# kakaobrain/rq-vae-transformer

Hardware: AMD Instinct MI355X
Metric: 256x256 images/sec, AR sampling + decode (RQ-Transformer huge, 8x8x4 codes) (higher is better)
Workload: dtype bf16

## Files before the change

### rq-vae-transformer_amd/csrc/conv_halo.hip

```cpp
#include <stdlib.h>
#include <type_traits>
#include "gemm.h"
#include "rq_common.h"
#include "vae_kernels.h"
#ifndef RQ_CONV_NT
#define RQ_CONV_NT 0
#endif
#ifndef RQ_CONVOUT_NT
#define RQ_CONVOUT_NT 0
#endif
static __device__ __forceinline__ rq_u128 ld128_act(const void* p) {
#if RQ_CONV_NT >= 2
    return ld128_nt(p);
#else
    return ld128(p);
#endif
}
static __device__ __forceinline__ void st128_act(void* p, rq_u128 v) {
#if RQ_CONV_NT >= 1
    st128_nt(p, v);
#else
    st128(p, v);
#endif
}

struct ConvHaloArgs {
    const bf16_t* x;
    const bf16_t* w;
    const float* bias;
    const float* gn;
    const bf16_t* resid;
    bf16_t* out;
    float* stats;
    int B, H, W, Cin, Cout;
};

#define RQ_LOG2E 1.4426950408889634f
static __device__ __forceinline__ float rq_silu_l2(float t) { return t * rq_fast_rcp(fmaf(rq_fast_exp2(-t), RQ_LOG2E, RQ_LOG2E)); }

static __device__ __forceinline__ void rq_stats_piece(const rq_u128& u, float (&sum)[4], float (&sq)[4]) {
    const uint32_t w[4] = {u.x, u.y, u.z, u.w};
#pragma unroll
    for (int e = 0; e < 4; ++e) {
        sum[e] = rq_dot2_bf16(w[e], RQ_ONE_X2, sum[e]);
        sq[e] = rq_dot2_bf16(w[e], w[e], sq[e]);
    }
}

constexpr int HT_H = 8, HT_W = 32;
constexpr int HP_W = HT_W + 2;
constexpr int H_BN = 128;
constexpr int HW_BYTES = H_BN * 128;
#ifndef RQ_HALO_WDMA
#define RQ_HALO_WDMA 1
#endif
#ifndef RQ_HALO_PMID
#define RQ_HALO_PMID 0
#endif
#ifndef RQ_HALO_RMID
#define RQ_HALO_RMID 1
#endif
#ifndef RQ_HALO_RES_F32
#define RQ_HALO_RES_F32 1
#endif
constexpr int H_WSLOTS = RQ_HALO_WDMA ? 4 : 3;
constexpr int H_SMEM_BYTES = 2 * (HT_H + 2) * HP_W * 128 + H_WSLOTS * HW_BYTES;
static __device__ __forceinline__ void halo_wait_dma(int nd, int no) {
#define RQ_HC(ND, K) case K: rq_wait_vmcnt_mixed<ND, K>(); break;
#define RQ_HW(ND) switch (no) { RQ_HC(ND, 0) RQ_HC(ND, 1) RQ_HC(ND, 2) RQ_HC(ND, 3) RQ_HC(ND, 4) RQ_HC(ND, 5) RQ_HC(ND, 6) RQ_HC(ND, 7) RQ_HC(ND, 8) \
    RQ_HC(ND, 9) RQ_HC(ND, 10) RQ_HC(ND, 11) RQ_HC(ND, 12) default: rq_wait_vmcnt_mixed<ND, 0>(); break; }
    if (nd >= 2) { RQ_HW(2) } else { RQ_HW(0) }
#undef RQ_HW
#undef RQ_HC
}

template <int PW = HP_W>
static __device__ __forceinline__ unsigned halo_lds_off(int hy, int hx, int c8) {
    return (unsigned)((hy * PW + hx) * 128 + ((c8 ^ ((hx >> 1) & 7)) << 4));
}

#ifdef RQ_CONV_TRACE
__device__ unsigned long long g_conv_trace[8 * 64];
#define RQ_CT(slot) do { if (blockIdx.x == RQ_CONV_TRACE && lane == 0 && (slot) < 64) g_conv_trace[wave * 64 + (slot)] = __builtin_readcyclecounter(); } while (0)
#else
#define RQ_CT(slot) do { } while (0)
#endif
template <int FUSE_GN, int UPS, int RES>
__global__ __launch_bounds__(512, 1) void conv3x3_halo_kernel(ConvHaloArgs p) {
    constexpr bool WDMA = RQ_HALO_WDMA != 0;
    constexpr int TH = HT_H, NTH = 512, RPW = 2, NJ = 2, W_IT = 2, TPX = TH * HT_W, W_SETS = 3, W_SLOTS = H_WSLOTS;
    static_assert(!(FUSE_GN && UPS), "the upsample conv has no Normalize in front of it");
    constexpr int PW = UPS ? HT_W / 2 + 2 : HP_W, PH = UPS ? TH / 2 + 2 : TH + 2;
    constexpr int HP_N = PW * PH;
    constexpr int HALO_BYTES = HP_N * 128;
    constexpr int H_IT = (HP_N * 8 + NTH - 1) / NTH;
    RQ_DYN_SMEM(smem);
    char* sH = (char*)smem;
    char* sW = sH + 2 * HALO_BYTES;
    const int tid = threadIdx.x, lane = tid & 63, wave = tid >> 6;
    const int wm = wave >> 1, wn = wave & 1;
#ifdef RQ_CONV_TRACE
    if (blockIdx.x == RQ_CONV_TRACE && lane == 0) g_conv_trace[wave * 64 + 58] = __builtin_amdgcn_s_memrealtime();
#endif

    const int tiles_x = p.W / HT_W, tiles_y = p.H / TH, NT = p.Cout / H_BN;
    const int n_mt = p.B * tiles_y * tiles_x;
    const int id = blockIdx.x, xcd = id & 7, slot = id >> 3;
    const int per = (n_mt + 7) >> 3;
    const int mtile = xcd * per + slot / NT;
    const int nt = slot - (slot / NT) * NT;
    if (slot >= per * NT || mtile >= n_mt) return;
    const int img = mtile / (tiles_y * tiles_x);
    const int trem = mtile - img * (tiles_y * tiles_x);
    const int ty0 = (trem / tiles_x) * TH, tx0 = (trem - (trem / tiles_x) * tiles_x) * HT_W;
    const int n0 = nt * H_BN;

    const char* gX = (const char*)p.x;
    const char* gWt = (const char*)p.w;
    const int w_row = tid >> 3, w_c8 = tid & 7;
    unsigned w_goff[W_IT];
#pragma unroll
    for (int i = 0; i < W_IT; ++i) w_goff[i] = (unsigned)(((long)(n0 + w_row + (NTH / 8) * i) * 9 * p.Cin + w_c8 * 8) * 2);
    auto load_w = [&](int c, int tap, rq_u128* rw) {
        const unsigned kb = (unsigned)(tap * p.Cin + c * 64) * 2u;
#pragma unroll
        for (int i = 0; i < W_IT; ++i) rw[i] = ld128(gWt + (w_goff[i] + kb));
    };
    rq_u128 rh[H_IT], rw[W_SETS][W_IT], r01[2][W_IT];
    unsigned w_voff[2];
#pragma unroll
    for (int i = 0; i < 2; ++i) {
        const int r = wave * 16 + i * 8 + (lane >> 3);
        w_voff[i] = (unsigned)(((long)(n0 + r) * 9 * p.Cin + ((lane & 7) ^ ((r >> 1) & 7)) * 8) * 2);
    }
    const rq_lds_t sW_dma = rq_lds_addr(sW) + (rq_lds_t)rq_uniform(wave) * 2048u;
    auto dma_w = [&](int c, int tap, unsigned woff) {
        if (tap >= 9) { tap -= 9; ++c; }
        rq_glds16_s2(sW_dma + woff, gWt + (unsigned)rq_uniform((tap * p.Cin + c * 64) * 2), w_voff[0], w_voff[1]);
    };
    if (WDMA) {
        dma_w(0, 0, 0u);
        dma_w(0, 1, (unsigned)HW_BYTES);
        dma_w(0, 2, 2u * HW_BYTES);
    } else {
        load_w(0, 0, r01[0]);
        load_w(0, 1, r01[1]);
        load_w(0, 2, rw[2]);
        load_w(0, 3, rw[0]);
        load_w(0, 4, rw[1]);
    }
    rq_sched_barrier();

    unsigned hd[H_IT];
    const int Hs = UPS ? p.H >> 1 : p.H, Ws = UPS ? p.W >> 1 : p.W;
    const unsigned x_img = (unsigned)((long)img * Hs * Ws * p.Cin * 2) + (unsigned)((tid & 7) * 16);
    const unsigned cin2 = (unsigned)p.Cin * 2u;
    const int hp0 = tid >> 3, hy0 = hp0 / PW, hx0 = hp0 - hy0 * PW;
    {
        int hy = hy0, hx = hx0;
#pragma unroll
        for (int it = 0; it < H_IT; ++it) {
            const int gy = (UPS ? ty0 >> 1 : ty0) + hy - 1, gx = (UPS ? tx0 >> 1 : tx0) + hx - 1;
            const int cy = gy < 0 ? 0 : (gy >= Hs ? Hs - 1 : gy), cx = gx < 0 ? 0 : (gx >= Ws ? Ws - 1 : gx);
            hd[it] = (unsigned)(cy * Ws + cx);
            rh[it] = ld128_act(gX + (x_img + hd[it] * cin2));
            hy += (NTH / 8) / PW; hx += (NTH / 8) % PW;
            if (hx >= PW) { hx -= PW; ++hy; }
        }
    }
    const float* gn = FUSE_GN ? p.gn + (long)img * p.Cin * 2 : nullptr;
    f32x4 gs[4];
    auto load_gs = [&](int c) {
        if (FUSE_GN) {
#pragma unroll
            for (int e = 0; e < 4; ++e) gs[e] = *(const f32x4*)(gn + (c * 64 + (tid & 7) * 8 + e * 2) * 2);
        }
    };
    auto scale_gs = [&]() {
        if (FUSE_GN) {
#pragma unroll
            for (int e = 0; e < 4; ++e) { rq_opaque_f4(gs[e]); gs[e] = gs[e] * RQ_LOG2E; }
        }
    };
    load_gs(0);
    rq_sched_barrier();
    {
        int hp = hp0, hy = hy0, hx = hx0;
        const int c8 = tid & 7;
#pragma unroll
        for (int it = 0; it < H_IT; ++it) {
            const bool in = hp < HP_N;
            const int gy = (UPS ? ty0 >> 1 : ty0) + hy - 1, gx = (UPS ? tx0 >> 1 : tx0) + hx - 1;
            const bool ok = in && gy >= 0 && gy < Hs && gx >= 0 && gx < Ws;
            const unsigned loff16 = in ? halo_lds_off<PW>(hy, hx, c8) >> 4 : 0u;
            hd[it] |= (loff16 << 16) | (ok ? 1u << 29 : 0u) | (in ? 1u << 30 : 0u);
            hp += NTH / 8; hy += (NTH / 8) / PW; hx += (NTH / 8) % PW;
            if (hx >= PW) { hx -= PW; ++hy; }
        }
    }
    auto h_in = [&](int it) { return (hd[it] >> 30) & 1u; };
    auto h_ok = [&](int it) { return (hd[it] >> 29) & 1u; };
    auto h_loff = [&](int it) { return ((hd[it] >> 16) & 0x1fffu) << 4; };
    auto h_goff = [&](int it) { return x_img + (hd[it] & 0xffffu) * cin2; };
    auto load_halo_piece = [&](int c, rq_u128* rh, int it) { rh[it] = ld128_act(gX + (h_goff(it) + (unsigned)c * 128u)); };

    unsigned w_loff[W_IT];
#pragma unroll
    for (int i = 0; i < W_IT; ++i) {
        const int r = w_row + (NTH / 8) * i;
        w_loff[i] = (unsigned)(r * 128 + ((w_c8 ^ ((r >> 1) & 7)) << 4));
    }
    auto halo_piece_value = [&](const rq_u128* rh, int it) -> rq_u128 {
        rq_u128 v = rh[it];
        if (FUSE_GN) {
            float f[8];
            rq_unpack2(v.x, f[0], f[1]);
            rq_unpack2(v.y, f[2], f[3]);
            rq_unpack2(v.z, f[4], f[5]);
            rq_unpack2(v.w, f[6], f[7]);
#pragma unroll
            for (int e = 0; e < 8; e += 2) {
                const f32x4 ss = gs[e >> 1];
                const float a = fmaf(f[e], ss[0], ss[1]), b = fmaf(f[e + 1], ss[2], ss[3]);
                f[e] = rq_silu_l2(a);
                f[e + 1] = rq_silu_l2(b);
            }
            v.x = pack_bf16x2(f[0], f[1]); v.y = pack_bf16x2(f[2], f[3]);
            v.z = pack_bf16x2(f[4], f[5]); v.w = pack_bf16x2(f[6], f[7]);
        }
        if (!h_ok(it)) v = zero128();
        return v;
    };
    auto halo_word = [&](rq_u128* rh, int it, int e) -> uint32_t& { return e == 0 ? rh[it].x : e == 1 ? rh[it].y : e == 2 ? rh[it].z : rh[it].w; };
    auto halo_piece_word = [&](rq_u128* rh, int it, int e) {
        uint32_t& w = halo_word(rh, it, e);
        if (FUSE_GN) {
            const f32x4 ss = gs[e];
            float wlo, whi;
            rq_unpack2(w, wlo, whi);
            const float a = fmaf(wlo, ss[0], ss[1]), b = fmaf(whi, ss[2], ss[3]);
            w = pack_bf16x2(rq_silu_l2(a), rq_silu_l2(b));
        }
        if (!h_ok(it)) w = 0u;
    };
    auto store_w = [&](int wslot, const rq_u128* rw) {
#pragma unroll
        for (int i = 0; i < W_IT; ++i) st128(sW + wslot * HW_BYTES + w_loff[i], rw[i]);
    };

    f32x16 acc[RPW][NJ];
#pragma unroll
    for (int j = 0; j < NJ; ++j)
#pragma unroll
        for (int q = 0; q < 4; ++q) {
            const f32x4 bv = *(const f32x4*)(p.bias + n0 + wn * (NJ * 32) + j * 32 + 8 * q + 4 * (lane >> 5));
#pragma unroll
            for (int i = 0; i < RPW; ++i)
#pragma unroll
                for (int e = 0; e < 4; ++e) acc[i][j][4 * q + e] = bv[e];
        }

    const int ftx = lane & 31, fk = lane >> 5;
    const unsigned rd_w0 = (unsigned)((wn * (NJ * 32) + ftx) * 128 + ((fk ^ ((ftx >> 1) & 7)) << 4));
    unsigned rd_h0[3];
#pragma unroll
    for (int kx = 0; kx < 3; ++kx)
        rd_h0[kx] = UPS ? halo_lds_off<PW>(wm * (RPW / 2), (ftx + kx + 1) >> 1, fk) : halo_lds_off<PW>(wm * RPW, ftx + kx, fk);

    auto load_frags = [&](int hbuf, unsigned woff, int ky, int kx, int ks, bf16x8* af, bf16x8* bfr) {
        const char* hb = sH + ((rd_h0[kx] + (unsigned)(hbuf * HALO_BYTES)) ^ (unsigned)(ks << 5));
        const char* wb = sW + ((rd_w0 ^ (unsigned)(ks << 5)) + woff);
#pragma unroll
        for (int i = 0; i < RPW; ++i) af[i] = as_bf16x8(ld128(hb + (UPS ? (i + ky + 1) >> 1 : i + ky) * (PW * 128)));
#pragma unroll
        for (int j = 0; j < NJ; ++j) bfr[j] = as_bf16x8(ld128(wb + j * (32 * 128)));
    };
#ifndef RQ_HALO_FDEPTH
#define RQ_HALO_FDEPTH 1
#endif
    constexpr int FD = RQ_HALO_FDEPTH, NSET = FD + 1;
    static_assert(FD >= 1 && FD <= 3 && 36 % NSET == 0, "fragment read-ahead of 1..3 k-steps");
    bf16x8 fa[NSET][RPW], fb[NSET][NJ];
    auto mfma_step = [&](int set) {
#pragma unroll
        for (int i = 0; i < RPW; ++i)
#pragma unroll
            for (int j = 0; j < NJ; ++j) acc[i][j] = rq_mfma_32x32x16_bf16(fb[set][j], fa[set][i], acc[i][j]);
    };

    const int NC = p.Cin / 64, last_c = NC - 1;
    auto load_unit = [&](int c, int tap, rq_u128* r) {
        if (tap >= 9) { tap -= 9; ++c; }
        if (c > last_c) return false;
        load_w(c, tap, r);
        return true;
    };
    {
        RQ_CT(0);
        scale_gs();
#pragma unroll
        for (int it = 0; it < H_IT; ++it)
            if (h_in(it)) st128(sH + h_loff(it), halo_piece_value(rh, it));
        if (WDMA) rq_wait_vmcnt_mixed<0, 0>();
        else {
            store_w(0, r01[0]);
            store_w(1, r01[1]);
        }
    }
    rq_syncthreads();
    RQ_CT(1);
#pragma unroll
    for (int g = 0; g < FD; ++g) load_frags(0, 0u, 0, 0, g, fa[g], fb[g]);
    constexpr int CPR = H_BN / 8;
    constexpr int R_IT = TPX * CPR / NTH;
    static_assert(R_IT == 8, "two residual pieces per tap in the first four taps of the last chunk");
    rq_u128 rr[R_IT];
    const bf16_t* rsrc = p.resid;
    static_assert(CPR == 16 && NTH / CPR == HT_W && R_IT == TH, "piece k = tile row k");
    const unsigned io_off0 = (unsigned)((((long)img * p.H + ty0) * p.W + tx0 + (tid >> 4)) * p.Cout + n0 + (tid & 15) * 8) * 2u;
    const unsigned io_step = (unsigned)p.W * (unsigned)p.Cout * 2u;
    auto run_chunk = [&](int c, auto last_tag) {
        constexpr bool LAST = decltype(last_tag)::value;
        const int hbuf = c & 1;
        const unsigned cph = (unsigned)c & 3u;
        auto slot_off = [&](int tap) { return WDMA ? ((cph + (unsigned)tap) & 3u) * (unsigned)HW_BYTES : (unsigned)((tap % 3) * HW_BYTES); };
        constexpr int NPT = H_IT, FIRST = 8 - NPT;
        static_assert(FIRST >= 0, "one patch piece per tap");
#pragma unroll
        for (int tap = 0; tap < 9; ++tap) {
            const int ky = tap / 3, kx = tap - ky * 3;
            const bool have_w2 = !(LAST && tap + 2 >= 9), have_w3 = !(LAST && tap + 3 >= 9);
#ifndef RQ_CONV_ABLATE_STAGE
            if (!WDMA && have_w2) store_w((tap + 2) % 3, rw[(tap + 2) % W_SETS]);
#endif
            if (!WDMA && have_w2) (void)load_unit(c, tap + 5, rw[(tap + 2) % W_SETS]);
            auto n_patch = [&](int t) {
                int n = 0;
                if (!LAST && t >= 0) {
                    if (t == 0 && FUSE_GN) n += 4;
#pragma unroll
                    for (int it = 0; it < H_IT; ++it) n += ((FIRST + it >= 3 ? FIRST + it - 3 : 0) == t) ? 1 : 0;
                }
                return n;
            };
            auto n_resid = [&](int t) { return LAST && RES && t >= 0 && t < R_IT / 2 ? 2 : 0; };
            auto patch_loads = [&]() {
                if (!LAST) {
                    if (tap == 0) load_gs(c + 1);
#pragma unroll
                    for (int it = 0; it < H_IT; ++it) {
                        const int t_use = FIRST + it, t_load = t_use >= 3 ? t_use - 3 : 0;
                        if (t_load == tap) load_halo_piece(c + 1, rh, it);
                    }
                }
            };
            auto resid_loads = [&]() {
                if (LAST && RES && tap < R_IT / 2) {
                    rr[2 * tap] = ld128_act((const char*)rsrc + (io_off0 + (unsigned)(2 * tap) * io_step));
                    rr[2 * tap + 1] = ld128_act((const char*)rsrc + (io_off0 + (unsigned)(2 * tap + 1) * io_step));
                }
            };
            constexpr bool PMID = WDMA && RQ_HALO_PMID, RMID = WDMA && RQ_HALO_RMID;
            if (!PMID) patch_loads();
            if (!RMID) resid_loads();
            const int n_vis = n_patch(tap) + n_resid(tap) + (PMID ? n_patch(tap - 1) : 0) + (RMID ? n_resid(tap - 1) : 0);
            if (!LAST && tap == 1) scale_gs();
            rq_sched_barrier();
            const int pit = tap - FIRST;
            const bool ptap = !LAST && pit >= 0 && pit < H_IT;
            const int pi = ptap ? pit : 0;
#pragma unroll
            for (int ks = 0; ks < 4; ++ks) {
#ifdef RQ_CONV_ABLATE_LDS
                if (false) {}
                else
#endif
#pragma unroll
                for (int i = 0; i < RPW; ++i)
#pragma unroll
                    for (int j = 0; j < NJ; ++j) rq_opaque_acc(acc[i][j]);
                {
                    const int g = tap * 4 + ks + FD, t2 = g >> 2, k2 = g & 3, set2 = g % NSET;
                    if (t2 < 9) load_frags(hbuf, slot_off(t2), t2 / 3, t2 % 3, k2, fa[set2], fb[set2]);
                    else if (!LAST) load_frags(hbuf ^ 1, slot_off(t2), (t2 - 9) / 3, (t2 - 9) % 3, k2, fa[set2], fb[set2]);
                }
                mfma_step((tap * 4 + ks) % NSET);
                if (FUSE_GN && ptap) rq_opaque_u(halo_word(rh, pi, ks));
                if (ptap) halo_piece_word(rh, pi, ks);
                if (FUSE_GN && ptap) rq_opaque_u(halo_word(rh, pi, ks));
                rq_sched_group(0x100, RPW + NJ);
#pragma unroll
                for (int m = 0; m < RPW * NJ; ++m) {
                    rq_sched_group(0x008, 1);
                    if (FUSE_GN && ptap) { rq_sched_group(0x002, 3); rq_sched_group(0x400, 1); }
                }
                rq_sched_barrier();
                if (WDMA && ks == 0) {
                    if (have_w3) dma_w(c, tap + 3, slot_off(tap + 3));
                    if (PMID) patch_loads();
                    if (RMID) resid_loads();
                    rq_sched_barrier();
                }
            }
            if (ptap) { if (h_in(pi)) st128(sH + (hbuf ^ 1) * HALO_BYTES + h_loff(pi), rh[pi]); }
            if (WDMA && have_w2) halo_wait_dma(have_w3 ? 2 : 0, n_vis);
            RQ_CT(2 + (c * 9 + tap) * 2);
            rq_syncthreads();
            RQ_CT(3 + (c * 9 + tap) * 2);
        }
    };
    for (int c = 0; c + 1 < NC; ++c) run_chunk(c, std::false_type{});
    run_chunk(NC - 1, std::true_type{});

    constexpr int LDR = H_BN * 2 + 16;
    static_assert(TPX * LDR + 4096 <= 160 * 1024, "epilogue tile must fit the CU's LDS (the launcher allocates max(staging, epilogue))");
    char* sT = (char*)smem;
    constexpr bool RF32 = RES && RQ_HALO_RES_F32;
    constexpr int LDF = H_BN * 4 + 16;
    static_assert(!RF32 || TPX * LDF <= H_SMEM_BYTES, "the fp32 tile overlays the operand buffers");
    if (RF32) {
#pragma unroll
        for (int i = 0; i < RPW; ++i) {
            const int ml = (wm * RPW + i) * HT_W + (lane & 31);
#pragma unroll
            for (int j = 0; j < NJ; ++j)
#pragma unroll
                for (int q = 0; q < 4; ++q) {
                    const int u = wn * (NJ * 8) + j * 8 + 2 * q + (lane >> 5);
                    f32x4 v;
#pragma unroll
                    for (int e = 0; e < 4; ++e) v[e] = acc[i][j][4 * q + e];
                    *(f32x4*)(sT + ml * LDF + ((u >> 1) + 16 * (u & 1)) * 16) = v;
                }
        }
    }
    if (RES && !RF32) {
#pragma unroll
        for (int k = 0; k < R_IT; ++k) st128(sT + ((tid >> 4) + HT_W * k) * LDR + (tid & 15) * 16, rr[k]);
        rq_syncthreads();
    }
    uint32_t rres[RPW][NJ][4][2];
    if (RES && !RF32) {
#pragma unroll
        for (int i = 0; i < RPW; ++i)
#pragma unroll
            for (int j = 0; j < NJ; ++j)
#pragma unroll
                for (int q = 0; q < 4; ++q) {
                    const int ml = (wm * RPW + i) * HT_W + (lane & 31);
                    const int nl = wn * (NJ * 32) + j * 32 + 8 * q + 4 * (lane >> 5);
                    const uint32_t* rp = (const uint32_t*)(sT + ml * LDR + nl * 2);
                    rres[i][j][q][0] = rp[0];
                    rres[i][j][q][1] = rp[1];
                }
        rq_sched_barrier();
    }
    if (!RF32)
#pragma unroll
    for (int i = 0; i < RPW; ++i) {
        const int ty = wm * RPW + i, tx = lane & 31;
        const int ml = ty * HT_W + tx;
#pragma unroll
        for (int j = 0; j < NJ; ++j) {
#pragma unroll
            for (int q = 0; q < 4; ++q) {
                const int nl = wn * (NJ * 32) + j * 32 + 8 * q + 4 * (lane >> 5);
                float v[4];
#pragma unroll
                for (int e = 0; e < 4; ++e) v[e] = acc[i][j][4 * q + e];
                if (RES && !RF32) {
                    const uint32_t r0 = rres[i][j][q][0], r1 = rres[i][j][q][1];
                    { float lo_, hi_; rq_unpack2(r0, lo_, hi_); v[0] += lo_; v[1] += hi_; }
                    { float lo_, hi_; rq_unpack2(r1, lo_, hi_); v[2] += lo_; v[3] += hi_; }
                }
                struct __attribute__((aligned(8))) u64 { uint32_t a, b; } w2;
                w2.a = pack_bf16x2(v[0], v[1]);
                w2.b = pack_bf16x2(v[2], v[3]);
                *(u64*)(sT + ml * LDR + nl * 2) = w2;
            }
        }
    }
    rq_syncthreads();
    RQ_CT(61);
    float gs_[4], gq_[4];
#pragma unroll
    for (int e = 0; e < 4; ++e) { gs_[e] = 0.f; gq_[e] = 0.f; }
#pragma unroll
    for (int k = 0; k < R_IT; ++k) {
        rq_u128 u;
        if (RF32) {
            const char* src = sT + ((tid >> 4) + HT_W * k) * LDF + (tid & 15) * 16;
            f32x4 a = *(const f32x4*)src, b = *(const f32x4*)(src + 256);
            const rq_u128 r = rr[k];
            { float lo_, hi_; rq_unpack2(r.x, lo_, hi_); a[0] += lo_; a[1] += hi_; }
            { float lo_, hi_; rq_unpack2(r.y, lo_, hi_); a[2] += lo_; a[3] += hi_; }
            { float lo_, hi_; rq_unpack2(r.z, lo_, hi_); b[0] += lo_; b[1] += hi_; }
            { float lo_, hi_; rq_unpack2(r.w, lo_, hi_); b[2] += lo_; b[3] += hi_; }
            u.x = pack_bf16x2(a[0], a[1]); u.y = pack_bf16x2(a[2], a[3]);
            u.z = pack_bf16x2(b[0], b[1]); u.w = pack_bf16x2(b[2], b[3]);
        } else {
            u = ld128(sT + ((tid >> 4) + HT_W * k) * LDR + (tid & 15) * 16);
        }
        st128_act((char*)p.out + (io_off0 + (unsigned)k * io_step), u);
        if (p.stats) rq_stats_piece(u, gs_, gq_);
    }
    if (p.stats) {
        __shared__ float sred[NTH / 64][16][4];
        const int gsz = p.Cout / 32;
        float a0, q0, a1, q1;
        if (gsz == 4) {
            a0 = gs_[0] + gs_[1]; q0 = gq_[0] + gq_[1];
            a1 = gs_[2] + gs_[3]; q1 = gq_[2] + gq_[3];
        } else {
            a0 = (gs_[0] + gs_[1]) + (gs_[2] + gs_[3]);
            q0 = (gq_[0] + gq_[1]) + (gq_[2] + gq_[3]);
            a1 = 0.f; q1 = 0.f;
        }
        a0 += rq_shfl_xor(a0, 16); q0 += rq_shfl_xor(q0, 16); a1 += rq_shfl_xor(a1, 16); q1 += rq_shfl_xor(q1, 16);
        a0 += rq_shfl_xor(a0, 32); q0 += rq_shfl_xor(q0, 32); a1 += rq_shfl_xor(a1, 32); q1 += rq_shfl_xor(q1, 32);
        if (lane < 16) { sred[wave][lane][0] = a0; sred[wave][lane][1] = q0; sred[wave][lane][2] = a1; sred[wave][lane][3] = q1; }
        rq_syncthreads();
        if (wave == 0) {
            const int chunk = (lane >> 1) & 15, pair = lane & 1;
            float a = 0.f, q = 0.f;
#pragma unroll
            for (int w = 0; w < NTH / 64; ++w) { a += sred[w][chunk][pair * 2]; q += sred[w][chunk][pair * 2 + 1]; }
            if (gsz == 16) {
                a += rq_shfl_xor(a, 2);
                q += rq_shfl_xor(q, 2);
            }
            const bool writer = gsz == 4 ? true : (gsz == 8 ? pair == 0 : (pair == 0 && (chunk & 1) == 0));
            if (writer && lane < 32) {
                const int g = (n0 + chunk * 8 + pair * 4) / gsz;
                const int tiles = tiles_x * tiles_y;
                float* o = p.stats + (((long)img * tiles + trem) * 32 + g) * 2;
                o[0] = a;
                o[1] = q;
            }
        }
    }
    RQ_CT(63);
#ifdef RQ_CONV_TRACE
    if (blockIdx.x == RQ_CONV_TRACE && lane == 0) g_conv_trace[wave * 64 + 59] = __builtin_amdgcn_s_memrealtime();
#endif
}

constexpr int PK_SMEM = 160 * 1024;
constexpr int PK_PATCH = (HT_H + 2) * HP_W * 128;
constexpr int PK_P0 = 2 * HW_BYTES;
constexpr int PK_P1 = PK_SMEM - PK_PATCH;
constexpr int PK_PSTRIDE = PK_P1 - PK_P0;
constexpr int PK_LDR = H_BN * 2 + 16;
constexpr int PK_TILE = HT_H * HT_W * PK_LDR;
constexpr int PK_RED = 8 * 16 * 4 * 4;
static_assert(PK_P0 + PK_PATCH + PK_TILE + PK_RED <= PK_SMEM, "epilogue tile over spare + P1");
static_assert(PK_P0 + PK_TILE + PK_RED <= PK_P1, "epilogue tile over P0 + spare");

struct HaloTile { int img, ty0, tx0, n0, trem, cls; };

template <int FUSE_GN, int UPS, int RES>
__global__ __launch_bounds__(512, 1) void conv3x3_halo_pk_kernel(ConvHaloArgs p, int wpx) {
    constexpr int TH = HT_H, NTH = 512, RPW = 2, W_IT = 2, TPX = TH * HT_W;
    constexpr bool SUB = UPS == 2;
    constexpr int TAPS = SUB ? 4 : 9, W_SETS = SUB ? 4 : 3;
    static_assert(!(FUSE_GN && UPS), "the upsample conv has no Normalize in front of it");
    constexpr int PW = UPS == 1 ? HT_W / 2 + 2 : HP_W, PH = UPS == 1 ? TH / 2 + 2 : TH + 2;
    constexpr int HP_N = PW * PH;
    constexpr int H_IT = (HP_N * 8 + NTH - 1) / NTH;
    RQ_DYN_SMEM(smem);
    char* sW = (char*)smem;
    char* sH = (char*)smem + PK_P0;
    const int tid = threadIdx.x, lane = tid & 63, wave = tid >> 6;
    const int wm = wave >> 1, wn = wave & 1;

    const int tiles_x = (SUB ? p.W >> 1 : p.W) / HT_W, tiles_y = (SUB ? p.H >> 1 : p.H) / TH, NT = p.Cout / H_BN;
    constexpr int NCLS = SUB ? 4 : 1;
    const int n_mt = p.B * tiles_y * tiles_x * NCLS;
    const int xcd = blockIdx.x & 7, w0 = blockIdx.x >> 3;
    const int per = (n_mt + 7) >> 3, nslot = per * NT;
    auto slot_ok = [&](int s) { return s < nslot && xcd * per + s / NT < n_mt; };
    auto decode = [&](int s) {
        HaloTile t;
        const int mtile = xcd * per + s / NT;
        t.n0 = (s - (s / NT) * NT) * H_BN;
        const int st = SUB ? mtile >> 2 : mtile;
        t.cls = SUB ? mtile & 3 : 0;
        t.img = st / (tiles_y * tiles_x);
        const int trem = st - t.img * (tiles_y * tiles_x);
        t.trem = trem * NCLS + t.cls;
        t.ty0 = (trem / tiles_x) * TH;
        t.tx0 = (trem - (trem / tiles_x) * tiles_x) * HT_W;
        return t;
    };
    int slot = w0;
    if (!slot_ok(slot)) return;

    unsigned hd[H_IT];
    unsigned x_img = 0;
    const float* gn = nullptr;
    const int Hs = UPS ? p.H >> 1 : p.H, Ws = UPS ? p.W >> 1 : p.W;
    auto set_staging = [&](const HaloTile& t) {
        int tid_s = tid;
        rq_opaque(tid_s);
#pragma unroll
        for (int it = 0; it < H_IT; ++it) {
            const int q = tid_s + NTH * it;
            const int hp = q >> 3, c8 = q & 7;
            const bool in = hp < HP_N;
            const int hy = hp / PW, hx = hp - hy * PW;
            const int gy = (UPS == 1 ? t.ty0 >> 1 : t.ty0) + hy - 1, gx = (UPS == 1 ? t.tx0 >> 1 : t.tx0) + hx - 1;
            const bool ok = in && gy >= 0 && gy < Hs && gx >= 0 && gx < Ws;
            const int cy = gy < 0 ? 0 : (gy >= Hs ? Hs - 1 : gy), cx = gx < 0 ? 0 : (gx >= Ws ? Ws - 1 : gx);
            const unsigned loff16 = in ? halo_lds_off<PW>(hy, hx, c8) >> 4 : 0u;
            hd[it] = (unsigned)(cy * Ws + cx) | (loff16 << 16) | (ok ? 1u << 29 : 0u) | (in ? 1u << 30 : 0u);
        }
        x_img = (unsigned)((long)t.img * Hs * Ws * p.Cin * 2) + (unsigned)((tid & 7) * 16);
        if (FUSE_GN) gn = p.gn + (long)t.img * p.Cin * 2;
    };
    auto restage = [&](const HaloTile& t) {
        int tid_s = tid;
        rq_opaque(tid_s);
        int hp = tid_s >> 3, hy = hp / PW, hx = hp - hy * PW;
#pragma unroll
        for (int it = 0; it < H_IT; ++it) {
            const unsigned in = (hd[it] >> 30) & 1u, lo = hd[it] & 0x1fff0000u;
            const int gy = (UPS == 1 ? t.ty0 >> 1 : t.ty0) + hy - 1, gx = (UPS == 1 ? t.tx0 >> 1 : t.tx0) + hx - 1;
            const bool ok = in && gy >= 0 && gy < Hs && gx >= 0 && gx < Ws;
            const int cy = gy < 0 ? 0 : (gy >= Hs ? Hs - 1 : gy), cx = gx < 0 ? 0 : (gx >= Ws ? Ws - 1 : gx);
// ... 666 lines not shown
bool rq_conv_in_mfma_supported(int H, int W, int Cin, int Cout) {
    return Cin == 3 && Cout == CI_COUT && H % HT_H == 0 && W % HT_W == 0;
}

int rq_launch_conv_in_mfma(const float* x, const float* w, const float* bias, bf16_t* y, float* stats, int B, int H, int W, hipStream_t s) {
    ConvInArgs a{};
    a.x = x; a.w = w; a.bias = bias; a.y = y; a.stats = stats; a.B = B; a.H = H; a.W = W;
    const size_t smem = 4096 + 128 + (size_t)CI_COUT * CI_WROW + 4 * (size_t)CI_STG;
    static RqDeviceOnce attr_once;
    if (attr_once.first()) {
        (void)hipFuncSetAttribute((const void*)conv_in_mfma_kernel, hipFuncAttributeMaxDynamicSharedMemorySize, (int)smem);
    }
    RQ_LAUNCH(conv_in_mfma_kernel, dim3((unsigned)(B * (H / HT_H) * (W / HT_W))), dim3(256), smem, s, a);
    return rq_check_launch("conv_in_mfma_kernel");
}

__global__ __launch_bounds__(256) void gn_params_kernel(const float* part, const float* gamma, const float* beta, float* gn, int B, int HW,
                                                        int C, int nchunk, float eps) {
    __shared__ float sa[8][32], sq[8][32], smean[32], srstd[32];
    const int b = blockIdx.x, tid = threadIdx.x, g = tid & 31, sl = tid >> 5;
    float a = 0.f, q = 0.f;
    for (int c = sl; c < nchunk; c += 8) {
        const float* o = part + (((long)b * nchunk + c) * 32 + g) * 2;
        a += o[0];
        q += o[1];
    }
    sa[sl][g] = a;
    sq[sl][g] = q;
    rq_syncthreads();
    if (tid < 32) {
        float ta = 0.f, tq = 0.f;
#pragma unroll
        for (int k = 0; k < 8; ++k) { ta += sa[k][tid]; tq += sq[k][tid]; }
        const float n = (float)HW * (float)(C / 32);
        const float mean = ta / n;
        float var = tq / n - mean * mean;
        if (var < 0.f) var = 0.f;
        smean[tid] = mean;
        srstd[tid] = 1.0f / sqrtf(var + eps);
    }
    rq_syncthreads();
    const int cpg = C / 32;
    for (int ch = tid; ch < C; ch += 256) {
        const int gg = ch / cpg;
        const float sc = srstd[gg] * gamma[ch];
        gn[((long)b * C + ch) * 2] = sc;
        gn[((long)b * C + ch) * 2 + 1] = beta[ch] - smean[gg] * sc;
    }
}

__global__ void ups_subpixel_weights_kernel(const bf16_t* w, bf16_t* wsub, int Cout, int Cin) {
    const long n = (long)4 * Cout * 4 * Cin;
    const long gid = (long)blockIdx.x * blockDim.x + threadIdx.x;
    if (gid >= n) return;
    const int ci = (int)(gid % Cin);
    long r = gid / Cin;
    const int tap = (int)(r & 3); r >>= 2;
    const int co = (int)(r % Cout);
    const int cls = (int)(r / Cout);
    const int py = cls >> 1, px = cls & 1, a = tap >> 1, b = tap & 1;
    const int ky_lo = py == 0 ? (a == 0 ? 0 : 1) : (a == 0 ? 0 : 2), ky_hi = py == 0 ? (a == 0 ? 0 : 2) : (a == 0 ? 1 : 2);
    const int kx_lo = px == 0 ? (b == 0 ? 0 : 1) : (b == 0 ? 0 : 2), kx_hi = px == 0 ? (b == 0 ? 0 : 2) : (b == 0 ? 1 : 2);
    float acc = 0.f;
    for (int ky = ky_lo; ky <= ky_hi; ++ky)
        for (int kx = kx_lo; kx <= kx_hi; ++kx) acc += bf16_to_f32(w[(((long)co * 3 + ky) * 3 + kx) * Cin + ci]);
    wsub[gid] = f32_to_bf16(acc);
}
int rq_launch_ups_subpixel_weights(const bf16_t* w, bf16_t* wsub, int Cout, int Cin, hipStream_t s) {
    const long n = (long)16 * Cout * Cin;
    RQ_LAUNCH(ups_subpixel_weights_kernel, dim3((unsigned)((n + 255) / 256)), dim3(256), 0, s, w, wsub, Cout, Cin);
    return rq_check_launch("ups_subpixel_weights_kernel");
}
bool rq_conv_halo_subpixel_supported(int H, int W, int Cin, int Cout) {
    return rq_conv_halo_supported(H, W, Cin, Cout) && (H >> 1) % HT_H == 0 && (W >> 1) % HT_W == 0;
}

bool rq_conv_halo_supported(int H, int W, int Cin, int Cout) {
    return H % HT_H == 0 && W % HT_W == 0 && Cin % 64 == 0 && Cout % H_BN == 0 && H >= 32 && H * W <= 65536;
}

int rq_conv_halo_stat_tiles(int H, int W) { return (H / HT_H) * (W / HT_W); }
static int g_conv_halo_dbg_pk = 0;
static int g_conv_halo_dbg_wpx = 0;
static bool halo_persistent(int ups) {
    static const int env = getenv("RQAMD_HALO_PERSIST") ? atoi(getenv("RQAMD_HALO_PERSIST")) : -1;
    if (g_conv_halo_dbg_pk) return g_conv_halo_dbg_pk > 0;
    return env < 0 ? ups != 0 : env != 0;
}

static int launch_conv_halo_th(const ConvHaloArgs& a, int ups, hipStream_t s) {
    constexpr int TH = HT_H, NTHR = 512;
    constexpr size_t smem = H_SMEM_BYTES;
    static_assert((size_t)TH * HT_W * (H_BN * 2 + 16) + 4096 <= H_SMEM_BYTES, "the epilogue tile overlays the operand buffers");
    static RqDeviceOnce attr_once;
    if (attr_once.first()) {
        (void)hipFuncSetAttribute((const void*)conv3x3_halo_kernel<0, 0, 0>, hipFuncAttributeMaxDynamicSharedMemorySize, (int)smem);
        (void)hipFuncSetAttribute((const void*)conv3x3_halo_kernel<0, 0, 1>, hipFuncAttributeMaxDynamicSharedMemorySize, (int)smem);
        (void)hipFuncSetAttribute((const void*)conv3x3_halo_kernel<1, 0, 0>, hipFuncAttributeMaxDynamicSharedMemorySize, (int)smem);
        (void)hipFuncSetAttribute((const void*)conv3x3_halo_kernel<1, 0, 1>, hipFuncAttributeMaxDynamicSharedMemorySize, (int)smem);
        (void)hipFuncSetAttribute((const void*)conv3x3_halo_kernel<0, 1, 0>, hipFuncAttributeMaxDynamicSharedMemorySize, (int)smem);
    }
    const int n_mt = a.B * (a.H / TH) * (a.W / HT_W), NT = a.Cout / H_BN;
    const int nblocks = 8 * ((n_mt + 7) / 8) * NT;
    if (ups == 2) {
        static RqDeviceOnce sub_once;
        static int cus_per_xcd_s[16];
        int dev = 0;
        (void)hipGetDevice(&dev);
        if (sub_once.first()) {
            (void)hipFuncSetAttribute((const void*)conv3x3_halo_pk_kernel<0, 2, 0>, hipFuncAttributeMaxDynamicSharedMemorySize, PK_SMEM);
            int cus = 0;
            if (hipDeviceGetAttribute(&cus, hipDeviceAttributeMultiprocessorCount, dev) != hipSuccess || cus < 8) cus = 256;
            cus_per_xcd_s[dev & 15] = cus / 8;
        }
        const int n_sub = a.B * ((a.H >> 1) / TH) * ((a.W >> 1) / HT_W) * 4;
        const int slots = ((n_sub + 7) / 8) * NT;
        int wpx = g_conv_halo_dbg_wpx > 0 ? g_conv_halo_dbg_wpx : cus_per_xcd_s[dev & 15];
        if (wpx > slots) wpx = slots;
        RQ_LAUNCH((conv3x3_halo_pk_kernel<0, 2, 0>), dim3(8 * wpx), dim3(512), PK_SMEM, s, a, wpx);
        return rq_check_launch("conv3x3_halo_pk_kernel<subpixel>");
    }
    if (ups && halo_persistent(ups)) {
        static RqDeviceOnce pk_once;
        static int cus_per_xcd[16];
        int dev = 0;
        (void)hipGetDevice(&dev);
        if (pk_once.first()) {
            (void)hipFuncSetAttribute((const void*)conv3x3_halo_pk_kernel<0, 1, 0>, hipFuncAttributeMaxDynamicSharedMemorySize, PK_SMEM);
            int cus = 0;
            if (hipDeviceGetAttribute(&cus, hipDeviceAttributeMultiprocessorCount, dev) != hipSuccess || cus < 8) cus = 256;
            cus_per_xcd[dev & 15] = cus / 8;
        }
        const int slots = ((n_mt + 7) / 8) * NT;
        int wpx = g_conv_halo_dbg_wpx > 0 ? g_conv_halo_dbg_wpx : cus_per_xcd[dev & 15];
        if (wpx > slots) wpx = slots;
        RQ_LAUNCH((conv3x3_halo_pk_kernel<0, 1, 0>), dim3(8 * wpx), dim3(512), PK_SMEM, s, a, wpx);
        return rq_check_launch("conv3x3_halo_pk_kernel");
    }
    if (ups) RQ_LAUNCH((conv3x3_halo_kernel<0, 1, 0>), dim3(nblocks), dim3(NTHR), smem, s, a);
    else if (a.gn && a.resid) RQ_LAUNCH((conv3x3_halo_kernel<1, 0, 1>), dim3(nblocks), dim3(NTHR), smem, s, a);
    else if (a.gn) RQ_LAUNCH((conv3x3_halo_kernel<1, 0, 0>), dim3(nblocks), dim3(NTHR), smem, s, a);
    else if (a.resid) RQ_LAUNCH((conv3x3_halo_kernel<0, 0, 1>), dim3(nblocks), dim3(NTHR), smem, s, a);
    else RQ_LAUNCH((conv3x3_halo_kernel<0, 0, 0>), dim3(nblocks), dim3(NTHR), smem, s, a);
    return rq_check_launch("conv3x3_halo_kernel");
}

int rq_launch_conv_halo(const bf16_t* x, const bf16_t* w, const float* bias, const float* gn, const bf16_t* resid, bf16_t* out,
                        float* stats, int B, int H, int W, int Cin, int Cout, int ups, hipStream_t s) {
    if (stats && Cout != 128 && Cout != 256 && Cout != 512) return rq_fail(RQAMD_ERR_UNSUPPORTED, "conv_halo: fused statistics need Cout 128/256/512");
    if (!rq_conv_halo_supported(H, W, Cin, Cout)) return rq_fail(RQAMD_ERR_UNSUPPORTED, "conv_halo: shape %dx%d %d->%d", H, W, Cin, Cout);
    if (ups && (gn || resid)) return rq_fail(RQAMD_ERR_UNSUPPORTED, "conv_halo: the upsample conv takes no GroupNorm / residual");
    if (ups == 2 && !rq_conv_halo_subpixel_supported(H, W, Cin, Cout)) return rq_fail(RQAMD_ERR_UNSUPPORTED, "conv_halo: sub-pixel form at %dx%d", H, W);
    if (2.0 * B * H * W * (Cin > Cout ? Cin : Cout) >= 4294967296.0) return rq_fail(RQAMD_ERR_UNSUPPORTED, "conv_halo: tensor larger than 4 GiB");
    ConvHaloArgs a{};
    a.x = x; a.w = w; a.bias = bias; a.gn = gn; a.resid = resid; a.out = out; a.stats = stats; a.B = B; a.H = H; a.W = W; a.Cin = Cin; a.Cout = Cout;
    return launch_conv_halo_th(a, ups, s);
}

int rq_launch_gn_params(const bf16_t* x, float* part, const float* gamma, const float* beta, float* gn, int B, int HW, int C,
                        int nchunk_have, hipStream_t s) {
    int nchunk = nchunk_have;
    if (nchunk <= 0) RQ_TRY(rq_launch_gn_stats(x, part, B, HW, C, &nchunk, s));
    RQ_LAUNCH(gn_params_kernel, dim3(B), dim3(256), 0, s, part, gamma, beta, gn, B, HW, C, nchunk, 1e-6f);
    return rq_check_launch("gn_params_kernel");
}

extern "C" int rqamd_dbg_conv_halo_bf16(const void* x, const void* w, const float* bias, const float* gn, const void* resid,
                                        int B, int H, int W, int Cin, int Cout, int ups, void* out, float* stats, void* stream) {
    if (!x || !w || !bias || !out) return rq_fail(RQAMD_ERR_INVALID, "dbg_conv_halo: null argument");
    g_conv_halo_dbg_pk = (ups & 16) ? 1 : (ups & 32) ? -1 : 0;
    g_conv_halo_dbg_wpx = (ups >> 8) & 0xff;
    const int rc = rq_launch_conv_halo((const bf16_t*)x, (const bf16_t*)w, bias, gn, (const bf16_t*)resid, (bf16_t*)out, stats, B, H, W,
                                       Cin, Cout, (ups & 64) ? 2 : (ups & 1), (hipStream_t)stream);
    g_conv_halo_dbg_pk = 0;
    g_conv_halo_dbg_wpx = 0;
    return rc;
}

extern "C" int rqamd_dbg_ups_subpixel_weights(const void* w, int Cout, int Cin, void* wsub, void* stream) {
    if (!w || !wsub) return rq_fail(RQAMD_ERR_INVALID, "dbg_ups_subpixel_weights: null argument");
    return rq_launch_ups_subpixel_weights((const bf16_t*)w, (bf16_t*)wsub, Cout, Cin, (hipStream_t)stream);
}

extern "C" int rqamd_dbg_conv_out_bf16(const void* x, const float* w, const float* bias, const float* gn, int B, int H, int W,
                                       int Cin, int Cout, float* y, void* stream) {
    if (!x || !w || !bias || !y) return rq_fail(RQAMD_ERR_INVALID, "dbg_conv_out: null argument");
    return rq_launch_conv_out_halo((const bf16_t*)x, w, bias, gn, y, B, H, W, Cin, Cout, (hipStream_t)stream);
}

extern "C" int rqamd_dbg_conv_in_bf16(const float* x, const float* w, const float* bias, int B, int H, int W, void* y, void* stream) {
    if (!x || !w || !bias || !y) return rq_fail(RQAMD_ERR_INVALID, "dbg_conv_in: null argument");
    if (!rq_conv_in_mfma_supported(H, W, 3, CI_COUT)) return rq_fail(RQAMD_ERR_UNSUPPORTED, "dbg_conv_in: shape %dx%d", H, W);
    return rq_launch_conv_in_mfma(x, w, bias, (bf16_t*)y, nullptr, B, H, W, (hipStream_t)stream);
}

#ifdef RQ_CONV_TRACE
extern "C" int rqamd_dbg_conv_trace(unsigned long long* out_host) {
    if (hipMemcpyFromSymbol(out_host, HIP_SYMBOL(g_conv_trace), sizeof(g_conv_trace)) != hipSuccess) return rq_fail(RQAMD_ERR_HIP, "conv_trace: copy failed");
    return RQAMD_OK;
}
#endif
```

Baseline: 1633.

## Add persistent fused GN conv3x3 kernel prefetching next tile across iterations

Turns the fused GroupNorm conv3x3 halo kernel into an optional persistent form. Each block loops over tiles strided by workers-per-XCD and, during the last chunk of the current tile, restages the halo and DMAs the first weight taps for the next tile. The epilogue is reworked into two half-tile passes so it fits inside a patch buffer while the next tile's prefetch is in flight. This is meant to hide per-tile startup latency and launch tail effects. The cost is much more control complexity, register pressure, and a changed residual load schedule. It is enabled by default for the fused non-upsample convs whose Cin/64 is even.

```diff
diff --git a/rq-vae-transformer_amd/csrc/conv_halo.hip b/rq-vae-transformer_amd/csrc/conv_halo.hip
--- a/rq-vae-transformer_amd/csrc/conv_halo.hip
+++ b/rq-vae-transformer_amd/csrc/conv_halo.hip
@@ -85,9 +85,10 @@
 #else
 #define RQ_CT(slot) do { } while (0)
 #endif
-template <int FUSE_GN, int UPS, int RES>
-__global__ __launch_bounds__(512, 1) void conv3x3_halo_kernel(ConvHaloArgs p) {
+template <int FUSE_GN, int UPS, int RES, bool PERSIST>
+static __device__ __forceinline__ void conv3x3_halo_body(const ConvHaloArgs& p, int wpx) {
     constexpr bool WDMA = RQ_HALO_WDMA != 0;
+    static_assert(!PERSIST || (WDMA && FUSE_GN && !UPS), "the persistent form is the fused conv on the LDS-DMA weight ring");
     constexpr int TH = HT_H, NTH = 512, RPW = 2, NJ = 2, W_IT = 2, TPX = TH * HT_W, W_SETS = 3, W_SLOTS = H_WSLOTS;
     static_assert(!(FUSE_GN && UPS), "the upsample conv has no Normalize in front of it");
     constexpr int PW = UPS ? HT_W / 2 + 2 : HP_W, PH = UPS ? TH / 2 + 2 : TH + 2;
@@ -105,15 +106,26 @@
 
     const int tiles_x = p.W / HT_W, tiles_y = p.H / TH, NT = p.Cout / H_BN;
     const int n_mt = p.B * tiles_y * tiles_x;
-    const int id = blockIdx.x, xcd = id & 7, slot = id >> 3;
+    const int id = blockIdx.x, xcd = id & 7;
+    int slot = id >> 3;
     const int per = (n_mt + 7) >> 3;
-    const int mtile = xcd * per + slot / NT;
-    const int nt = slot - (slot / NT) * NT;
-    if (slot >= per * NT || mtile >= n_mt) return;
-    const int img = mtile / (tiles_y * tiles_x);
-    const int trem = mtile - img * (tiles_y * tiles_x);
-    const int ty0 = (trem / tiles_x) * TH, tx0 = (trem - (trem / tiles_x) * tiles_x) * HT_W;
-    const int n0 = nt * H_BN;
+    auto slot_ok = [&](int s) { return s < per * NT && xcd * per + s / NT < n_mt; };
+    if (!slot_ok(slot)) return;
+    struct Tile { int img, trem, ty0, tx0, n0; };
+    auto decode = [&](int s) {
+        Tile t;
+        const int mtile = xcd * per + s / NT;
+        t.n0 = (s - (s / NT) * NT) * H_BN;
+        t.img = mtile / (tiles_y * tiles_x);
+        t.trem = mtile - t.img * (tiles_y * tiles_x);
+        t.ty0 = (t.trem / tiles_x) * TH;
+        t.tx0 = (t.trem - (t.trem / tiles_x) * tiles_x) * HT_W;
+        return t;
+    };
+    Tile cur = decode(slot);
+    int img = cur.img, trem = cur.trem, ty0 = cur.ty0, tx0 = cur.tx0, n0 = cur.n0;
+    bool has_next = PERSIST && slot_ok(slot + wpx);
+    Tile nxt = has_next ? decode(slot + wpx) : cur;
 
     const char* gX = (const char*)p.x;
     const char* gWt = (const char*)p.w;
@@ -131,12 +143,17 @@
 #pragma unroll
     for (int i = 0; i < 2; ++i) {
         const int r = wave * 16 + i * 8 + (lane >> 3);
-        w_voff[i] = (unsigned)(((long)(n0 + r) * 9 * p.Cin + ((lane & 7) ^ ((r >> 1) & 7)) * 8) * 2);
+        w_voff[i] = (unsigned)(((long)((PERSIST ? 0 : n0) + r) * 9 * p.Cin + ((lane & 7) ^ ((r >> 1) & 7)) * 8) * 2);
     }
     const rq_lds_t sW_dma = rq_lds_addr(sW) + (rq_lds_t)rq_uniform(wave) * 2048u;
+    auto w_base = [&](int nb) { return PERSIST ? (unsigned)nb * 9u * (unsigned)p.Cin * 2u : 0u; };
+    unsigned wb_cur = w_base(n0), wb_nxt = w_base(nxt.n0);
+    auto dma_w_at = [&](unsigned wb, int c, int tap, unsigned woff) {
+        rq_glds16_s2(sW_dma + woff, gWt + (unsigned)rq_uniform(wb + (unsigned)((tap * p.Cin + c * 64) * 2)), w_voff[0], w_voff[1]);
+    };
     auto dma_w = [&](int c, int tap, unsigned woff) {
         if (tap >= 9) { tap -= 9; ++c; }
-        rq_glds16_s2(sW_dma + woff, gWt + (unsigned)rq_uniform((tap * p.Cin + c * 64) * 2), w_voff[0], w_voff[1]);
+        dma_w_at(wb_cur, c, tap, woff);
     };
     if (WDMA) {
         dma_w(0, 0, 0u);
@@ -153,7 +170,7 @@
 
     unsigned hd[H_IT];
     const int Hs = UPS ? p.H >> 1 : p.H, Ws = UPS ? p.W >> 1 : p.W;
-    const unsigned x_img = (unsigned)((long)img * Hs * Ws * p.Cin * 2) + (unsigned)((tid & 7) * 16);
+    unsigned x_img = (unsigned)((long)img * Hs * Ws * p.Cin * 2) + (unsigned)((tid & 7) * 16);
     const unsigned cin2 = (unsigned)p.Cin * 2u;
     const int hp0 = tid >> 3, hy0 = hp0 / PW, hx0 = hp0 - hy0 * PW;
     {
@@ -203,6 +220,23 @@
     auto h_loff = [&](int it) { return ((hd[it] >> 16) & 0x1fffu) << 4; };
     auto h_goff = [&](int it) { return x_img + (hd[it] & 0xffffu) * cin2; };
     auto load_halo_piece = [&](int c, rq_u128* rh, int it) { rh[it] = ld128_act(gX + (h_goff(it) + (unsigned)c * 128u)); };
+    auto restage = [&](const Tile& t) {
+        int tid_s = tid;
+        rq_opaque(tid_s);
+        int hy = (tid_s >> 3) / PW, hx = (tid_s >> 3) - hy * PW;
+#pragma unroll
+        for (int it = 0; it < H_IT; ++it) {
+            const unsigned in = (hd[it] >> 30) & 1u, lo = hd[it] & 0x1fff0000u;
+            const int gy = t.ty0 + hy - 1, gx = t.tx0 + hx - 1;
+            const bool ok = in && gy >= 0 && gy < Hs && gx >= 0 && gx < Ws;
+            const int cy = gy < 0 ? 0 : (gy >= Hs ? Hs - 1 : gy), cx = gx < 0 ? 0 : (gx >= Ws ? Ws - 1 : gx);
+            hd[it] = (unsigned)(cy * Ws + cx) | lo | (ok ? 1u << 29 : 0u) | (in << 30);
+            hy += (NTH / 8) / PW; hx += (NTH / 8) % PW;
+            if (hx >= PW) { hx -= PW; ++hy; }
+        }
+        x_img = (unsigned)((long)t.img * Hs * Ws * p.Cin * 2) + (unsigned)((tid_s & 7) * 16);
+        gn = p.gn + (long)t.img * p.Cin * 2;
+    };
 
     unsigned w_loff[W_IT];
 #pragma unroll
@@ -249,16 +283,19 @@
     };
 
     f32x16 acc[RPW][NJ];
-#pragma unroll
-    for (int j = 0; j < NJ; ++j)
-#pragma unroll
-        for (int q = 0; q < 4; ++q) {
-            const f32x4 bv = *(const f32x4*)(p.bias + n0 + wn * (NJ * 32) + j * 32 + 8 * q + 4 * (lane >> 5));
-#pragma unroll
-            for (int i = 0; i < RPW; ++i)
-#pragma unroll
-                for (int e = 0; e < 4; ++e) acc[i][j][4 * q + e] = bv[e];
-        }
+    auto acc_from_bias = [&](int nb) {
+#pragma unroll
+        for (int j = 0; j < NJ; ++j)
+#pragma unroll
+            for (int q = 0; q < 4; ++q) {
+                const f32x4 bv = *(const f32x4*)(p.bias + nb + wn * (NJ * 32) + j * 32 + 8 * q + 4 * (lane >> 5));
+#pragma unroll
+                for (int i = 0; i < RPW; ++i)
+#pragma unroll
+                    for (int e = 0; e < 4; ++e) acc[i][j][4 * q + e] = bv[e];
+            }
+    };
+    acc_from_bias(n0);
 
     const int ftx = lane & 31, fk = lane >> 5;
     const unsigned rd_w0 = (unsigned)((wn * (NJ * 32) + ftx) * 128 + ((fk ^ ((ftx >> 1) & 7)) << 4));
@@ -317,57 +354,63 @@
     rq_u128 rr[R_IT];
     const bf16_t* rsrc = p.resid;
     static_assert(CPR == 16 && NTH / CPR == HT_W && R_IT == TH, "piece k = tile row k");
-    const unsigned io_off0 = (unsigned)((((long)img * p.H + ty0) * p.W + tx0 + (tid >> 4)) * p.Cout + n0 + (tid & 15) * 8) * 2u;
+    unsigned io_off0 = (unsigned)((((long)img * p.H + ty0) * p.W + tx0 + (tid >> 4)) * p.Cout + n0 + (tid & 15) * 8) * 2u;
     const unsigned io_step = (unsigned)p.W * (unsigned)p.Cout * 2u;
+    unsigned tph = 0u;
     auto run_chunk = [&](int c, auto last_tag) {
         constexpr bool LAST = decltype(last_tag)::value;
+        constexpr bool STG = !LAST || PERSIST;
         const int hbuf = c & 1;
-        const unsigned cph = (unsigned)c & 3u;
+        const int cn = LAST ? 0 : c + 1;
+        if constexpr (PERSIST && LAST) restage(nxt);
+        const unsigned cph = ((unsigned)c + tph) & 3u;
         auto slot_off = [&](int tap) { return WDMA ? ((cph + (unsigned)tap) & 3u) * (unsigned)HW_BYTES : (unsigned)((tap % 3) * HW_BYTES); };
         constexpr int NPT = H_IT, FIRST = 8 - NPT;
         static_assert(FIRST >= 0, "one patch piece per tap");
 #pragma unroll
         for (int tap = 0; tap < 9; ++tap) {
             const int ky = tap / 3, kx = tap - ky * 3;
-            const bool have_w2 = !(LAST && tap + 2 >= 9), have_w3 = !(LAST && tap + 3 >= 9);
+            const bool have_w2 = !(LAST && !PERSIST && tap + 2 >= 9), have_w3 = !(LAST && !PERSIST && tap + 3 >= 9);
 #ifndef RQ_CONV_ABLATE_STAGE
             if (!WDMA && have_w2) store_w((tap + 2) % 3, rw[(tap + 2) % W_SETS]);
 #endif
             if (!WDMA && have_w2) (void)load_unit(c, tap + 5, rw[(tap + 2) % W_SETS]);
             auto n_patch = [&](int t) {
                 int n = 0;
-                if (!LAST && t >= 0) {
+                if (STG && t >= 0) {
                     if (t == 0 && FUSE_GN) n += 4;
 #pragma unroll
                     for (int it = 0; it < H_IT; ++it) n += ((FIRST + it >= 3 ? FIRST + it - 3 : 0) == t) ? 1 : 0;
                 }
                 return n;
             };
-            auto n_resid = [&](int t) { return LAST && RES && t >= 0 && t < R_IT / 2 ? 2 : 0; };
+            constexpr int RT0 = PERSIST ? 4 : 0;
+            auto n_resid = [&](int t) { return LAST && RES && t >= RT0 && t < RT0 + R_IT / 2 ? 2 : 0; };
             auto patch_loads = [&]() {
-                if (!LAST) {
-                    if (tap == 0) load_gs(c + 1);
+                if (STG) {
+                    if (tap == 0) load_gs(cn);
 #pragma unroll
                     for (int it = 0; it < H_IT; ++it) {
                         const int t_use = FIRST + it, t_load = t_use >= 3 ? t_use - 3 : 0;
-                        if (t_load == tap) load_halo_piece(c + 1, rh, it);
+                        if (t_load == tap) load_halo_piece(cn, rh, it);
                     }
                 }
             };
             auto resid_loads = [&]() {
-                if (LAST && RES && tap < R_IT / 2) {
-                    rr[2 * tap] = ld128_act((const char*)rsrc + (io_off0 + (unsigned)(2 * tap) * io_step));
-                    rr[2 * tap + 1] = ld128_act((const char*)rsrc + (io_off0 + (unsigned)(2 * tap + 1) * io_step));
+                if (LAST && RES && tap >= RT0 && tap < RT0 + R_IT / 2) {
+                    const int k = 2 * (tap - RT0);
+                    rr[k] = ld128_act((const char*)rsrc + (io_off0 + (unsigned)k * io_step));
+                    rr[k + 1] = ld128_act((const char*)rsrc + (io_off0 + (unsigned)(k + 1) * io_step));
                 }
             };
             constexpr bool PMID = WDMA && RQ_HALO_PMID, RMID = WDMA && RQ_HALO_RMID;
             if (!PMID) patch_loads();
             if (!RMID) resid_loads();
             const int n_vis = n_patch(tap) + n_resid(tap) + (PMID ? n_patch(tap - 1) : 0) + (RMID ? n_resid(tap - 1) : 0);
-            if (!LAST && tap == 1) scale_gs();
+            if (STG && tap == 1) scale_gs();
             rq_sched_barrier();
             const int pit = tap - FIRST;
-            const bool ptap = !LAST && pit >= 0 && pit < H_IT;
+            const bool ptap = STG && pit >= 0 && pit < H_IT;
             const int pi = ptap ? pit : 0;
 #pragma unroll
             for (int ks = 0; ks < 4; ++ks) {
@@ -396,7 +439,8 @@
                 }
                 rq_sched_barrier();
                 if (WDMA && ks == 0) {
-                    if (have_w3) dma_w(c, tap + 3, slot_off(tap + 3));
+                    if (PERSIST && LAST && tap + 3 >= 9) dma_w_at(wb_nxt, 0, tap - 6, slot_off(tap + 3));
+                    else if (have_w3) dma_w(c, tap + 3, slot_off(tap + 3));
                     if (PMID) patch_loads();
                     if (RMID) resid_loads();
                     rq_sched_barrier();
@@ -409,9 +453,73 @@
             RQ_CT(3 + (c * 9 + tap) * 2);
         }
     };
+    for (;;) {
     for (int c = 0; c + 1 < NC; ++c) run_chunk(c, std::false_type{});
     run_chunk(NC - 1, std::true_type{});
 
+    float gs_[4], gq_[4];
+#pragma unroll
+    for (int e = 0; e < 4; ++e) { gs_[e] = 0.f; gq_[e] = 0.f; }
+    if constexpr (PERSIST) {
+        constexpr int LDR = H_BN * 2 + 16, HROWS = TH / 2;
+        static_assert(HROWS * HT_W * LDR <= HALO_BYTES && RPW * 2 == HROWS, "half an epilogue tile fits a patch buffer");
+        char* sT = sH + HALO_BYTES;
+#pragma unroll
+        for (int h = 0; h < 2; ++h) {
+            if (RES) {
+#pragma unroll
+                for (int k = 0; k < HROWS; ++k) st128(sT + ((tid >> 4) + HT_W * k) * LDR + (tid & 15) * 16, rr[HROWS * h + k]);
+                rq_syncthreads();
+            }
+            if ((wm >> 1) == h) {
+                uint32_t rres[RPW][NJ][4][2];
+                if (RES) {
+#pragma unroll
+                    for (int i = 0; i < RPW; ++i)
+#pragma unroll
+                        for (int j = 0; j < NJ; ++j)
+#pragma unroll
+                            for (int q = 0; q < 4; ++q) {
+                                const int ml = (wm * RPW + i - HROWS * h) * HT_W + (lane & 31);
+                                const int nl = wn * (NJ * 32) + j * 32 + 8 * q + 4 * (lane >> 5);
+                                const uint32_t* rp = (const uint32_t*)(sT + ml * LDR + nl * 2);
+                                rres[i][j][q][0] = rp[0];
+                                rres[i][j][q][1] = rp[1];
+                            }
+                    rq_sched_barrier();
+                }
+#pragma unroll
+                for (int i = 0; i < RPW; ++i) {
+                    const int ml = (wm * RPW + i - HROWS * h) * HT_W + (lane & 31);
+#pragma unroll
+                    for (int j = 0; j < NJ; ++j)
+#pragma unroll
+                        for (int q = 0; q < 4; ++q) {
+                            const int nl = wn * (NJ * 32) + j * 32 + 8 * q + 4 * (lane >> 5);
+                            float v[4];
+#pragma unroll
+                            for (int e = 0; e < 4; ++e) v[e] = acc[i][j][4 * q + e];
+                            if (RES) {
+                                { float lo_, hi_; rq_unpack2(rres[i][j][q][0], lo_, hi_); v[0] += lo_; v[1] += hi_; }
+                                { float lo_, hi_; rq_unpack2(rres[i][j][q][1], lo_, hi_); v[2] += lo_; v[3] += hi_; }
+                            }
+                            struct __attribute__((aligned(8))) u64 { uint32_t a, b; } w2;
+                            w2.a = pack_bf16x2(v[0], v[1]);
+                            w2.b = pack_bf16x2(v[2], v[3]);
+                            *(u64*)(sT + ml * LDR + nl * 2) = w2;
+                        }
+                }
+            }
+            rq_syncthreads();
+#pragma unroll
+            for (int k = 0; k < HROWS; ++k) {
+                const rq_u128 u = ld128(sT + ((tid >> 4) + HT_W * k) * LDR + (tid & 15) * 16);
+                st128_act((char*)p.out + (io_off0 + (unsigned)(HROWS * h + k) * io_step), u);
+                if (p.stats) rq_stats_piece(u, gs_, gq_);
+            }
+            if (h == 0) rq_syncthreads();
+        }
+    } else {
     constexpr int LDR = H_BN * 2 + 16;
     static_assert(TPX * LDR + 4096 <= 160 * 1024, "epilogue tile must fit the CU's LDS (the launcher allocates max(staging, epilogue))");
     char* sT = (char*)smem;
@@ -482,9 +590,6 @@
     }
     rq_syncthreads();
     RQ_CT(61);
-    float gs_[4], gq_[4];
-#pragma unroll
-    for (int e = 0; e < 4; ++e) { gs_[e] = 0.f; gq_[e] = 0.f; }
 #pragma unroll
     for (int k = 0; k < R_IT; ++k) {
         rq_u128 u;
@@ -504,6 +609,7 @@
         st128_act((char*)p.out + (io_off0 + (unsigned)k * io_step), u);
         if (p.stats) rq_stats_piece(u, gs_, gq_);
     }
+    }
     if (p.stats) {
         __shared__ float sred[NTH / 64][16][4];
         const int gsz = p.Cout / 32;
@@ -539,11 +645,38 @@
             }
         }
     }
+    if constexpr (!PERSIST) {
+        break;
+    } else {
+        if (!has_next) {
+            rq_wait_vmcnt_mixed<0, 0>();
+            break;
+        }
+        slot += wpx;
+        cur = nxt;
+        img = cur.img; trem = cur.trem; ty0 = cur.ty0; tx0 = cur.tx0; n0 = cur.n0;
+        tph = (tph + 9u * (unsigned)NC) & 3u;
+        wb_cur = wb_nxt;
+        has_next = slot_ok(slot + wpx);
+        nxt = has_next ? decode(slot + wpx) : cur;
+        wb_nxt = w_base(nxt.n0);
+        io_off0 = (unsigned)((((long)img * p.H + ty0) * p.W + tx0 + (tid >> 4)) * p.Cout + n0 + (tid & 15) * 8) * 2u;
+        acc_from_bias(n0);
+#pragma unroll
+        for (int g = 0; g < FD; ++g) load_frags(0, tph * (unsigned)HW_BYTES, 0, 0, g, fa[g], fb[g]);
+    }
+    }
     RQ_CT(63);
 #ifdef RQ_CONV_TRACE
     if (blockIdx.x == RQ_CONV_TRACE && lane == 0) g_conv_trace[wave * 64 + 59] = __builtin_amdgcn_s_memrealtime();
 #endif
 }
+
+template <int FUSE_GN, int UPS, int RES>
+__global__ __launch_bounds__(512, 1) void conv3x3_halo_kernel(ConvHaloArgs p) { conv3x3_halo_body<FUSE_GN, UPS, RES, false>(p, 0); }
+
+template <int RES>
+__global__ __launch_bounds__(512, 1) void conv3x3_halo_pd_kernel(ConvHaloArgs p, int wpx) { conv3x3_halo_body<1, 0, RES, true>(p, wpx); }
 
 constexpr int PK_SMEM = 160 * 1024;
 constexpr int PK_PATCH = (HT_H + 2) * HP_W * 128;
@@ -1376,10 +1509,13 @@
 int rq_conv_halo_stat_tiles(int H, int W) { return (H / HT_H) * (W / HT_W); }
 static int g_conv_halo_dbg_pk = 0;
 static int g_conv_halo_dbg_wpx = 0;
-static bool halo_persistent(int ups) {
+static bool halo_persistent(int ups, const ConvHaloArgs& a) {
     static const int env = getenv("RQAMD_HALO_PERSIST") ? atoi(getenv("RQAMD_HALO_PERSIST")) : -1;
+    const bool fused = !ups && a.gn;
+    if (fused && (a.Cin / 64) % 2 != 0) return false;
+    if (!ups && !fused) return false;
     if (g_conv_halo_dbg_pk) return g_conv_halo_dbg_pk > 0;
-    return env < 0 ? ups != 0 : env != 0;
+    return env < 0 || env != 0;
 }
 
 static int launch_conv_halo_th(const ConvHaloArgs& a, int ups, hipStream_t s) {
@@ -1414,7 +1550,26 @@
         RQ_LAUNCH((conv3x3_halo_pk_kernel<0, 2, 0>), dim3(8 * wpx), dim3(512), PK_SMEM, s, a, wpx);
         return rq_check_launch("conv3x3_halo_pk_kernel<subpixel>");
     }
-    if (ups && halo_persistent(ups)) {
+    if (!ups && halo_persistent(ups, a)) {
+        static RqDeviceOnce pd_once;
+        static int cus_per_xcd_d[16];
+        int dev = 0;
+        (void)hipGetDevice(&dev);
+        if (pd_once.first()) {
+            (void)hipFuncSetAttribute((const void*)conv3x3_halo_pd_kernel<0>, hipFuncAttributeMaxDynamicSharedMemorySize, (int)smem);
+            (void)hipFuncSetAttribute((const void*)conv3x3_halo_pd_kernel<1>, hipFuncAttributeMaxDynamicSharedMemorySize, (int)smem);
+            int cus = 0;
+            if (hipDeviceGetAttribute(&cus, hipDeviceAttributeMultiprocessorCount, dev) != hipSuccess || cus < 8) cus = 256;
+            cus_per_xcd_d[dev & 15] = cus / 8;
+        }
+        const int slots = ((n_mt + 7) / 8) * NT;
+        int wpx = g_conv_halo_dbg_wpx > 0 ? g_conv_halo_dbg_wpx : cus_per_xcd_d[dev & 15];
+        if (wpx > slots) wpx = slots;
+        if (a.resid) RQ_LAUNCH((conv3x3_halo_pd_kernel<1>), dim3(8 * wpx), dim3(NTHR), smem, s, a, wpx);
+        else RQ_LAUNCH((conv3x3_halo_pd_kernel<0>), dim3(8 * wpx), dim3(NTHR), smem, s, a, wpx);
+        return rq_check_launch("conv3x3_halo_pd_kernel");
+    }
+    if (ups && halo_persistent(ups, a)) {
         static RqDeviceOnce pk_once;
         static int cus_per_xcd[16];
         int dev = 0;
```

Result: faster. 1653 (median of 6 runs) (+1.2%).
